# yanconglin/ICP-Flow

Measured on AMD Instinct MI355X. Metric: cluster-pair ICP registrations/sec, higher is better.
Workload: dtype f32

## Files before the change

icp_flow_amd/csrc/api.hip:

```cpp
#include <stdarg.h>
#include <stdio.h>
#include <stdlib.h>
#include <string.h>

#include "kernels.hpp"
#include "posefuse.hpp"
#include "kabsch.hpp"
#include "host.hpp"

using namespace icpflow;

namespace {

thread_local char g_err[512] = "";

}

namespace icpflow {
int report_error(int code, const char *message)
{
    snprintf(g_err, sizeof(g_err), "%s", message);
    return code;
}

// ... 920 lines not shown
    io.estimateScale = o.estimateScale;
    io.initS = o.initS;
    if ((o.allowReflection || o.estimateScale) && o.arith != ICPFLOW_ARITH_FP64)
        return report_errorf(ICPFLOW_E_ARG, "icpflow_icp: allow_reflection / estimate_scale are not built for ICPFLOW_ARITH_FP32_REFERENCE");
    if (o.history != nullptr &&
        !(stop_mode == ICPFLOW_STOP_REFERENCE && max_iterations > 1 && max_iterations <= kHistIters &&
          o.arith == ICPFLOW_ARITH_FP64 && io.speculative))
        return report_errorf(ICPFLOW_E_ARG, "icpflow_icp: options.d_icp_history needs the single-launch reference stop mode "
                                            "(2 <= max_iterations <= %d, fp64 arithmetic)", kHistIters);
    if (o.initR != nullptr && o.arith != ICPFLOW_ARITH_FP64)
        return report_errorf(ICPFLOW_E_ARG, "icpflow_icp: an initial transform is not built for ICPFLOW_ARITH_FP32_REFERENCE");
    Opts os = o;
    if ((o.estimateScale || o.initS != nullptr) && o.search == 0 && N < 64) os.search = 3;
    const GridScratch *search = search_scratch(w, N, os);
    if ((o.estimateScale || o.initS != nullptr) && (search == nullptr || search->mode != 3))
        return report_errorf(ICPFLOW_E_ARG, "icpflow_icp: estimate_scale / an initial transform with a scale need the sorted-sweep "
                                            "search (the default up to N = %d)", kMaxSortN);
    launch_count_pair(d_X, d_Y, B, N, w.lenA, w.lenC, nullptr, s, w.ctrl, icp_ctrl_bytes(B));
    ICPFLOW_TRY(launch_icp(d_X, d_Y, w.lenA, w.lenC, nullptr, d_pre_pose, B, N, thres, max_iterations,
                           relative_rmse_thr, stop_mode, w.state, w.ctrl, search, w.history, &w.team,
                           io, s));
    if (o.history != nullptr)
        ICPFLOW_TRY(hipMemcpyAsync(o.history, w.history, (size_t)max_iterations * B * kHistStride * sizeof(float),
                                   hipMemcpyDeviceToDevice, s));
    ICPFLOW_TRY(launch_icp_export(w.state, w.ctrl, B, stop_mode, d_R, d_T, d_rmse, d_iters, d_converged, s, o.scaleOut));
    return 0;
}

int icpflow_apply_icp(const float *d_src, const float *d_dst, const float *d_init, int B, int N,
                      double thres_dist, int max_iterations, double relative_rmse_thr, int stop_mode,
                      float *d_T_out, int32_t *d_iters, void *d_ws, size_t ws_bytes,
                      icpflow_stream_t stream, const icpflow_options_t *opt)
{
    Opts o;
    if (int r = parse_options("icpflow_apply_icp", opt, o)) return r;
    if (int r = check_arith("icpflow_apply_icp", o, max_iterations, stop_mode)) return r;
    if (int r = check_pair_active("icpflow_apply_icp", o, false, max_iterations, stop_mode)) return r;
    if (!d_src || !d_dst || !d_init || !d_T_out) return report_errorf(ICPFLOW_E_ARG, "icpflow_apply_icp: null pointer");
    if (int r = check_batch("icpflow_apply_icp", B, N)) return r;
    if (max_iterations <= 0 || max_iterations > kMaxIterCap)
        return report_errorf(ICPFLOW_E_ARG, "icpflow_apply_icp: max_iterations must be in 1..%d", kMaxIterCap);
    if (stop_mode != ICPFLOW_STOP_REFERENCE && stop_mode != ICPFLOW_STOP_PER_PAIR)
        return report_errorf(ICPFLOW_E_ARG, "icpflow_apply_icp: unknown stop_mode %d", stop_mode);
    Workspace w(d_ws, B, N, 0);
    if (int r = check_ws(d_ws, ws_bytes, w.bytes)) return r;
    hipStream_t s = (hipStream_t)stream;
    launch_count_pair(d_src, d_dst, B, N, w.lenA, w.lenC, nullptr, s, w.ctrl, icp_ctrl_bytes(B));
    ICPFLOW_TRY(hipMemcpyAsync(w.Tinit, d_init, (size_t)B * 16 * sizeof(float), hipMemcpyDeviceToDevice, s));
    return run_icp_and_select(d_src, d_dst, w, nullptr, w.Tinit, B, N, thres_dist, max_iterations,
                              relative_rmse_thr, stop_mode, 0, d_T_out, d_iters, o, s);
}

static int hist_icp_core(const float *d_src, const float *d_dst, int B, int N, const float *d_edges_x, int len_x,
                         const float *d_edges_y, int len_y, const float *d_edges_z, int len_z, float decode_shift,
                         double thres_dist, int max_iterations, double relative_rmse_thr, int stop_mode,
                         float *d_T_out, int32_t *d_iters, Workspace &w, const Opts &o, hipStream_t s,
                         int phase = 0, int32_t *carry = nullptr)
{
    if (phase == 2) {
        w.grid.presorted = carry[0];
        w.grid.shareCountClean = 1;
        int32_t pending = carry[2];
        return run_icp_and_select(d_src, d_dst, w, w.swap, w.Tinit, B, N, thres_dist, max_iterations,
                                  relative_rmse_thr, stop_mode, 1, d_T_out, d_iters, o, s, carry[1] != 0, 2, &pending, carry[3] != 0);
    }
    const bool countInSort = N <= kMaxSortN && N <= kChunkSortMinN && o.on(ICPFLOW_OPT_NO_SORTED_VOTE);
    if (!countInSort) {
        launch_count_pair(d_src, d_dst, B, N, w.lenA, w.lenC, w.swap, s, w.ctrl, icp_ctrl_bytes(B), w.scoreAccum,
                          w.accumBytes, w.pairBox);
        w.grid.pairBox = w.pairBox;
    }
    hipEvent_t join = nullptr;
    bool teamPlanned = false;
    JoinGuard guard;
    const GridScratch *search = search_scratch(w, N, o);
    SideStream *side = nullptr;
    if (search != nullptr && search->mode == 3 && N >= 64 && o.on(ICPFLOW_OPT_NO_SIDE_STREAM)) {
        side = &side_stream(s);
        if (!side->ok) side = nullptr;
    }
    if (side != nullptr) {
        ICPFLOW_TRY(hipEventRecord(side->fork, s));
        ICPFLOW_TRY(hipStreamWaitEvent(side->stream, side->fork, 0));
        hipError_t se = launch_sort_clouds_soa(d_src, d_dst, w.lenA, w.lenC, w.swap, B, N, &w.grid, side->stream,
                                               countInSort ? 2 : 0);
        if (se == hipSuccess && score_by_sweep(N, true, o) && o.on(ICPFLOW_OPT_NO_SCORE_PRUNE) && o.on(ICPFLOW_OPT_NO_SCORE_PREBOUND)) {
            se = launch_occupancy(&w.grid, B, N, side->stream);
            if (se == hipSuccess) w.grid.occReady = 1;
        }
        if (se == hipSuccess && !countInSort && phase != 1 &&
            icp_teams_wanted(&w.team, o.icp(w.grid.sortX), search, B, N, max_iterations, stop_mode, w.history)) {
            launch_icp_team_plan(&w.team, w.lenA, w.lenC, w.swap, B, N, o.icp(w.grid.sortX), side->stream);
            teamPlanned = true;
        }
        const hipError_t je = hipEventRecord(side->join, side->stream);
        if (je == hipSuccess) { guard.s = s; guard.join = side->join; }
        ICPFLOW_TRY(se);
        ICPFLOW_TRY(je);
        w.grid.presorted = 1;
        join = side->join;
    }
    PairCountFuse fuse{};
    if (countInSort) {
        fuse.swapOut = w.swap;
        fuse.zero0 = w.ctrl; fuse.bytes0 = icp_ctrl_bytes(B);
        fuse.zero1 = w.scoreAccum; fuse.bytes1 = w.accumBytes;
    }
    w.grid.shareCountClean = 1;
    w.grid.sweepTicket = w.ticketScratch;
    const bool sweepScore = score_by_sweep(N, join != nullptr, o);
    if (int r = run_init_pose(d_src, d_dst, w, w.swap, B, N, d_edges_x, len_x, d_edges_y, len_y, d_edges_z,
                              len_z, decode_shift, w.Tinit, o, s, sweepScore ? join : nullptr,
                              countInSort ? &fuse : nullptr, join != nullptr))
        return r;
    if (join != nullptr && !sweepScore) ICPFLOW_TRY(hipStreamWaitEvent(s, join, 0));
    guard.joined();
    if (phase == 1) {
        carry[0] = w.grid.presorted;
        carry[1] = teamPlanned ? 1 : 0;
        carry[3] = w.initSumValid ? 1 : 0;
        return run_icp_and_select(d_src, d_dst, w, w.swap, w.Tinit, B, N, thres_dist, max_iterations, relative_rmse_thr,
                                  stop_mode, 1, d_T_out, d_iters, o, s, teamPlanned, 1, &carry[2]);
    }
    return run_icp_and_select(d_src, d_dst, w, w.swap, w.Tinit, B, N, thres_dist, max_iterations,
                              relative_rmse_thr, stop_mode, 1, d_T_out, d_iters, o, s, teamPlanned, 0, nullptr, w.initSumValid);
}

int icpflow_hist_icp(const float *d_src, const float *d_dst, int B, int N, const float *d_edges_x,
                     int len_x, const float *d_edges_y, int len_y, const float *d_edges_z, int len_z,
                     float decode_shift, double thres_dist, int max_iterations, double relative_rmse_thr,
                     int stop_mode, float *d_T_out, int32_t *d_iters, void *d_ws, size_t ws_bytes,
                     icpflow_stream_t stream, const icpflow_options_t *opt)
{
    Opts o;
    if (int r = parse_options("icpflow_hist_icp", opt, o)) return r;
    if (int r = check_arith("icpflow_hist_icp", o, max_iterations, stop_mode)) return r;
    if (int r = check_pair_active("icpflow_hist_icp", o, true, max_iterations, stop_mode)) return r;
    if (!d_src || !d_dst || !d_edges_x || !d_edges_y || !d_edges_z || !d_T_out)
        return report_errorf(ICPFLOW_E_ARG, "icpflow_hist_icp: null pointer");
    if (int r = check_batch("icpflow_hist_icp", B, N)) return r;
    if (int r = check_hist_dims("icpflow_hist_icp", len_x, len_y, len_z)) return r;
    if (max_iterations <= 0 || max_iterations > kMaxIterCap)
        return report_errorf(ICPFLOW_E_ARG, "icpflow_hist_icp: max_iterations must be in 1..%d", kMaxIterCap);
    if (stop_mode != ICPFLOW_STOP_REFERENCE && stop_mode != ICPFLOW_STOP_PER_PAIR)
        return report_errorf(ICPFLOW_E_ARG, "icpflow_hist_icp: unknown stop_mode %d", stop_mode);
    const size_t L = (size_t)len_x * len_y * len_z;
    if (L < (size_t)kTopK) return report_errorf(ICPFLOW_E_ARG, "icpflow_hist_icp: fewer than 5 bins");
    Workspace w(d_ws, B, N, L);
    if (int r = check_ws(d_ws, ws_bytes, w.bytes)) return r;
    return hist_icp_core(d_src, d_dst, B, N, d_edges_x, len_x, d_edges_y, len_y, d_edges_z, len_z, decode_shift,
                         thres_dist, max_iterations, relative_rmse_thr, stop_mode, d_T_out, d_iters, w, o,
                         (hipStream_t)stream);
}

int icpflow_hist_icp_many(int K, const float *const *d_src, const float *const *d_dst, const int *B, int N,
                          const float *d_edges_x, int len_x, const float *d_edges_y, int len_y,
                          const float *d_edges_z, int len_z, float decode_shift, double thres_dist,
                          int max_iterations, double relative_rmse_thr, int stop_mode, float *const *d_T_out,
                          int32_t *const *d_iters, void *const *d_ws, const size_t *ws_bytes,
                          icpflow_stream_t stream, const icpflow_options_t *opt)
{
    if (K <= 0 || K > 64) return report_errorf(ICPFLOW_E_ARG, "icpflow_hist_icp_many: K must be in 1..64 (got %d)", K);
    if (!d_src || !d_dst || !B || !d_T_out || !d_iters || !d_ws || !ws_bytes)
        return report_errorf(ICPFLOW_E_ARG, "icpflow_hist_icp_many: null pointer");
    for (int k = 0; k < K; ++k)
        for (int j = 0; j < k; ++j)
            if (d_ws[k] == d_ws[j]) return report_errorf(ICPFLOW_E_WORKSPACE, "icpflow_hist_icp_many: batches %d and %d share a workspace", j, k);
    hipStream_t s = (hipStream_t)stream;
    constexpr int kWorkers = 4;
// ... 160 lines not shown
```

icp_flow_amd/csrc/hist.hip:

```cpp
#include "common.hpp"
#include "kernels.hpp"
#include "votekey.hpp"

namespace icpflow {

__global__ __launch_bounds__(256) void count_valid_kernel(const float4 *__restrict__ pts, int N,
                                                          int32_t *__restrict__ len)
{
    __shared__ int scratch[4];
    const int b = blockIdx.x;
    const float4 *p = pts + (size_t)b * N;
    int c[1] = {0};
    for (int i = threadIdx.x; i < N; i += blockDim.x) c[0] += (p[i].w > 0.0f) ? 1 : 0;
    block_sum<1, int>(c, scratch);
    if (threadIdx.x == 0) len[b] = c[0];
}

__global__ __launch_bounds__(1024) void count_pair_kernel(const float4 *__restrict__ A, const float4 *__restrict__ C,
                                                         int N, int32_t *__restrict__ lenA,
                                                         int32_t *__restrict__ lenC, uint8_t *__restrict__ swap,
                                                         uint32_t *__restrict__ zero0, unsigned words0,
                                                         uint32_t *__restrict__ zero1, unsigned words1,
                                                         float *__restrict__ boxes)
{
// ... 595 lines not shown
    if (useLds && N > kVoteWideN && B <= kVoteWideB * cus) {
        dim3 grid(((N + 127) / 128) * tsplit, B);
        const int lspan = (work != nullptr && N >= ICPFLOW_VOTE_LIST_MIN_N) ? min(span, kVoteListSpan) : span;
        const int ltsplit = (N + lspan - 1) / lspan;
        const size_t U = (size_t)((N + 127) / 128) * ltsplit * B;
        const bool listed = work != nullptr && U <= workCap && B <= 1024 && (N + 127) / 128 <= 256 && ltsplit <= 128 &&
                            N >= ICPFLOW_VOTE_LIST_MIN_N;
        if (listed) {
            hipLaunchKernelGGL(vote_plan_kernel, dim3((unsigned)((U + 1023) / 1024)), dim3(1024), 0, s, nX, nY, swap, B, 128, lspan,
                               (int)U, work, orderOut);
            if (planned != nullptr) *planned = orderOut != nullptr;
            grid = dim3((unsigned)U, 1);
        }
        hipLaunchKernelGGL((hist_vote_sorted_kernel<512, 4>), grid, dim3(512), lds_hist, s,
                           (const float4 *)sortX, (const float4 *)sortY, nX, nY, N, lens[0], lens[1], lens[2], ex, ey,
                           ez, swap, useLds, bins_u32, keyRec, listed ? lspan : span, listed ? work : (const int32_t *)nullptr, B);
        return hipGetLastError();
    }
    if (block == 1024) {
        dim3 grid(((N + 1023) / 1024) * tsplit, B);
        hipLaunchKernelGGL(hist_vote_sorted_kernel<1024>, grid, dim3(1024), useLds ? lds_hist : tile_bytes, s,
                           (const float4 *)sortX, (const float4 *)sortY, nX, nY, N, lens[0], lens[1], lens[2], ex, ey,
                           ez, swap, useLds, bins_u32, keyRec, span, (const int32_t *)nullptr, B);
    } else if (block == 512 && !split) {
        dim3 grid(((N + 511) / 512) * tsplit, B);
        hipLaunchKernelGGL(hist_vote_sorted_kernel<512>, grid, dim3(512), useLds ? lds_hist : tile_bytes, s,
                           (const float4 *)sortX, (const float4 *)sortY, nX, nY, N, lens[0], lens[1], lens[2], ex, ey,
                           ez, swap, useLds, bins_u32, keyRec, span, (const int32_t *)nullptr, B);
    } else if (split) {
        dim3 grid(((N + kVoteBlock - 1) / kVoteBlock) * tsplit, B);
        hipLaunchKernelGGL((hist_vote_sorted_kernel<2 * kVoteBlock, 2>), grid, dim3(2 * kVoteBlock), lds_hist, s,
                           (const float4 *)sortX, (const float4 *)sortY, nX, nY, N, lens[0], lens[1], lens[2], ex, ey,
                           ez, swap, useLds, bins_u32, keyRec, span, (const int32_t *)nullptr, B);
    } else {
        dim3 grid(((N + kVoteBlock - 1) / kVoteBlock) * tsplit, B);
        hipLaunchKernelGGL(hist_vote_sorted_kernel<kVoteBlock>, grid, dim3(kVoteBlock), useLds ? lds_hist : tile_bytes, s,
                           (const float4 *)sortX, (const float4 *)sortY, nX, nY, N, lens[0], lens[1], lens[2], ex, ey,
                           ez, swap, useLds, bins_u32, keyRec, span, (const int32_t *)nullptr, B);
    }
    return hipGetLastError();
}

__global__ void u32_to_f32_kernel(const uint32_t *__restrict__ in, float *__restrict__ out, size_t n)
{
    const size_t i = (size_t)blockIdx.x * blockDim.x + threadIdx.x;
    if (i < n) out[i] = (float)in[i];
}

hipError_t launch_hist_vote(const float *X, const float *Y, int B, int NX, int NY,
                            const float mins[3], const float maxs[3], const int lens[3],
                            const float *ex, const float *ey, const float *ez,
                            const uint8_t *swap, uint32_t *bins_u32, hipStream_t s)
{
    VoteBox box{mins ? mins[0] : 0.f, mins ? mins[1] : 0.f, mins ? mins[2] : 0.f,
                maxs ? maxs[0] : 0.f, maxs ? maxs[1] : 0.f, maxs ? maxs[2] : 0.f,
                lens[0], lens[1], lens[2]};
    const size_t L = (size_t)lens[0] * lens[1] * lens[2];
    hipError_t e = hipMemsetAsync(bins_u32, 0, sizeof(uint32_t) * L * (size_t)B, s);
    if (e != hipSuccess) return e;
    const int rows = swap ? (NX > NY ? NX : NY) : NX;
    dim3 grid((rows + kVoteBlock - 1) / kVoteBlock, B);
    const size_t tile_bytes = sizeof(float4) * kVoteTile;
    const size_t lds_hist = tile_bytes + sizeof(uint32_t) * (L + (size_t)vote_overflow_bins(lens[1], lens[2]));
    if (lds_hist <= 64 * 1024) {
        hipLaunchKernelGGL(hist_vote_kernel<true>, grid, dim3(kVoteBlock), lds_hist, s,
                           (const float4 *)X, (const float4 *)Y, NX, NY, box, ex, ey, ez, swap,
                           bins_u32);
    } else {
        hipLaunchKernelGGL(hist_vote_kernel<false>, grid, dim3(kVoteBlock), tile_bytes, s,
                           (const float4 *)X, (const float4 *)Y, NX, NY, box, ex, ey, ez, swap,
                           bins_u32);
    }
    return hipGetLastError();
}

hipError_t launch_u32_to_f32(const uint32_t *in, float *out, size_t n, hipStream_t s)
{
    hipLaunchKernelGGL(u32_to_f32_kernel, dim3((unsigned)((n + 255) / 256)), dim3(256), 0, s, in, out, n);
    return hipGetLastError();
}

constexpr int kPeakBlock = 1024;
constexpr int kPeakMaxK = 8;

template <int R>
__device__ __forceinline__ uint32_t peak_window_max(const uint32_t *__restrict__ V, int f, int c, int n, int stride)
{
    uint32_t v[2 * R + 1];
#pragma unroll
    for (int dq = -R; dq <= R; ++dq) v[dq + R] = V[f + (min(max(c + dq, 0), n - 1) - c) * stride];
    uint32_t m = v[0];
#pragma unroll
    for (int u = 1; u < 2 * R + 1; ++u) m = max(m, v[u]);
    return m;
}

#ifdef ICPFLOW_PEAK_CLOCK
__device__ unsigned long long g_peakClock[1024][8];
#define PEAK_STAMP(k) do { if (threadIdx.x == 0 && blockIdx.x < 1024) g_peakClock[blockIdx.x][k] = wall_clock64(); } while (0)
#else
#define PEAK_STAMP(k) do { } while (0)
#endif
template <typename BinT, int MEM>
__global__ __launch_bounds__(kPeakBlock) void hist_peaks_kernel(
    const BinT *__restrict__ bins, int Lx, int Ly, int Lz, int k, int radius,
    uint32_t *__restrict__ wsA, uint32_t *__restrict__ wsB, float *__restrict__ votes,
    int64_t *__restrict__ idx_out, PeakDecode dec)
{
    extern __shared__ __attribute__((aligned(16))) unsigned char smem[];
    __shared__ unsigned long long red[(kPeakBlock / kWave) * kPeakMaxK];
    __shared__ unsigned long long chosen[kPeakMaxK];
    const int b = blockIdx.x;
    const int L = Lx * Ly * Lz;
    const BinT *h = bins + (size_t)b * L;
    uint32_t *H0 = reinterpret_cast<uint32_t *>(smem);
    uint32_t *A = MEM ? H0 + L : wsA + (size_t)b * L;
    uint32_t *Bv = MEM ? H0 + 2 * (size_t)L : wsB + (size_t)b * L;
    const int tid = threadIdx.x;
    PEAK_STAMP(0);
    if (MEM) {
        for (int f = tid; f < L; f += kPeakBlock) H0[f] = (uint32_t)h[f];
        __syncthreads();
    }
    PEAK_STAMP(1);
    const int LyLz = Ly * Lz;
    const int stepX = kPeakBlock / LyLz, stepY = (kPeakBlock % LyLz) / Lz, stepZ = kPeakBlock % Lz;
    const int x0 = tid / LyLz, y0 = (tid % LyLz) / Lz, z0 = tid % Lz;
#define ICPFLOW_PEAK_ADVANCE()                                   \
    do {                                                         \
        z += stepZ; y += stepY; x += stepX;                      \
        if (z >= Lz) { z -= Lz; ++y; }                           \
        if (y >= Ly) { y -= Ly; ++x; }                           \
    } while (0)
    {
        int x = x0, y = y0, z = z0;
        for (int f = tid; f < L; f += kPeakBlock) {
            (void)x;
            uint32_t m = 0;
            if (MEM && radius >= 2 && Lz == 3) m = max(max(H0[f - z], H0[f - z + 1]), H0[f - z + 2]);
            else {
                const int lo = max(0, z - radius), hi = min(Lz - 1, z + radius);
                for (int q = lo; q <= hi; ++q) m = max(m, MEM ? H0[f + (q - z)] : (uint32_t)h[f + (q - z)]);
            }
            A[f] = m;
            ICPFLOW_PEAK_ADVANCE();
        }
    }
    __syncthreads();
    PEAK_STAMP(2);
    {
        int x = x0, y = y0, z = z0;
        for (int f = tid; f < L; f += kPeakBlock) {
            (void)x;
            uint32_t m = 0;
            if (radius == 5) m = peak_window_max<5>(A, f, y, Ly, Lz);
            else {
                const int lo = max(0, y - radius), hi = min(Ly - 1, y + radius);
                for (int q = lo; q <= hi; ++q) m = max(m, A[f + (q - y) * Lz]);
            }
            Bv[f] = m;
            ICPFLOW_PEAK_ADVANCE();
        }
    }
    __syncthreads();
    PEAK_STAMP(3);
    {
        int x = x0, y = y0, z = z0;
        for (int f = tid; f < L; f += kPeakBlock) {
            uint32_t m = 0;
            if (radius == 5) m = peak_window_max<5>(Bv, f, x, Lx, LyLz);
            else {
                const int lo = max(0, x - radius), hi = min(Lx - 1, x + radius);
                for (int q = lo; q <= hi; ++q) m = max(m, Bv[f + (q - x) * LyLz]);
            }
            A[f] = m;
            ICPFLOW_PEAK_ADVANCE();
        }
    }
#undef ICPFLOW_PEAK_ADVANCE
    __syncthreads();
    PEAK_STAMP(4);
    const int lane = tid & (kWave - 1), wave = tid >> 6;
    unsigned long long *wtop = reinterpret_cast<unsigned long long *>(red);
    {
        unsigned long long below = ~0ull, best = 0ull;
        bool stale = true;
        for (int r = 0; r < k; ++r) {
            if (stale) {
                best = 0ull;
                for (int f = tid; f < L; f += kPeakBlock) {
                    const uint32_t v = MEM ? H0[f] : (uint32_t)h[f];
                    const uint32_t sv = (v == A[f]) ? v : 0u;
                    const unsigned long long key =
                        ((unsigned long long)sv << 32) | (unsigned long long)(0xFFFFFFFFu - (uint32_t)f);
                    if (key < below && key > best) best = key;
                }
                stale = false;
            }
            const unsigned long long w = wave_max_u64_dpp(best);
            if (lane == 0) wtop[wave * kPeakMaxK + r] = w;
            if (w == best && w != 0ull) { below = best; stale = true; }
        }
    }
    __syncthreads();
    PEAK_STAMP(5);
    if (wave == 0) {
        constexpr int kWaves = kPeakBlock / kWave;
        unsigned long long c0 = 0ull, c1 = 0ull;
        {
            const int n = kWaves * k;
            if (lane < n) c0 = wtop[(lane / k) * kPeakMaxK + lane % k];
            if (lane + kWave < n) c1 = wtop[((lane + kWave) / k) * kPeakMaxK + (lane + kWave) % k];
        }
        for (int r = 0; r < k; ++r) {
            const unsigned long long m = wave_max_u64_dpp(c0 > c1 ? c0 : c1);
            if (lane == 0) chosen[r] = m;
            if (c0 == m) c0 = 0ull;
            if (c1 == m) c1 = 0ull;
        }
    }
    __syncthreads();
    PEAK_STAMP(6);
    if (tid < k) {
        const int r = tid;
        const unsigned long long m = chosen[r];
        votes[(size_t)b * k + r] = (float)(uint32_t)(m >> 32);
        const uint32_t f = 0xFFFFFFFFu - (uint32_t)(m & 0xFFFFFFFFull);
        idx_out[(size_t)b * k + r] = (int64_t)f;
        if (dec.cand != nullptr) {
            float *o = dec.cand + ((size_t)b * (k + 1) + r) * 3;
            const int ix = (int)(f / Lz / Ly % Lx), iy = (int)(f / Lz % Ly), iz = (int)(f % Lz);
            o[0] = dec.ex[ix] + dec.shift; o[1] = dec.ey[iy] + dec.shift; o[2] = dec.ez[iz] + dec.shift;
            if (r == k - 1) { o[3] = 0.f; o[4] = 0.f; o[5] = 0.f; }
        }
    }
}

template <typename BinT>
static hipError_t launch_peaks_t(const BinT *bins, int B, int Lx, int Ly, int Lz, int k,
                                 int kernel_size, uint32_t *wsA, uint32_t *wsB, float *votes,
                                 int64_t *idx, PeakDecode dec, hipStream_t s)
{
    const size_t lds = 3 * sizeof(uint32_t) * (size_t)Lx * Ly * Lz;
    if (lds <= 150 * 1024) {
        static std::atomic<unsigned long long> attr{0ull};
        ensure_dynamic_lds(reinterpret_cast<const void *>(&hist_peaks_kernel<BinT, 1>), 150 * 1024, &attr);
        hipLaunchKernelGGL((hist_peaks_kernel<BinT, 1>), dim3(B), dim3(kPeakBlock), lds, s, bins, Lx, Ly, Lz, k,
                           (kernel_size - 1) / 2, wsA, wsB, votes, idx, dec);
    } else {
        hipLaunchKernelGGL((hist_peaks_kernel<BinT, 0>), dim3(B), dim3(kPeakBlock), 0, s, bins, Lx, Ly, Lz, k,
                           (kernel_size - 1) / 2, wsA, wsB, votes, idx, dec);
    }
    return hipGetLastError();
}

hipError_t launch_hist_peaks_f32(const float *bins, int B, int Lx, int Ly, int Lz, int k,
                                 int kernel_size, uint32_t *wsA, uint32_t *wsB, float *votes,
                                 int64_t *idx, hipStream_t s)
{
    return launch_peaks_t<float>(bins, B, Lx, Ly, Lz, k, kernel_size, wsA, wsB, votes, idx, PeakDecode{}, s);
}

hipError_t launch_hist_peaks_u32(const uint32_t *bins, int B, int Lx, int Ly, int Lz, int k,
                                 int kernel_size, uint32_t *wsA, uint32_t *wsB, float *votes,
                                 int64_t *idx, hipStream_t s, PeakDecode dec)
{
    return launch_peaks_t<uint32_t>(bins, B, Lx, Ly, Lz, k, kernel_size, wsA, wsB, votes, idx, dec, s);
}

}

#ifdef ICPFLOW_PEAK_CLOCK
extern "C" int icpflow_debug_peak_clock(unsigned long long *out)
{
    (void)hipDeviceSynchronize();
    return (int)hipMemcpyFromSymbol(out, HIP_SYMBOL(icpflow::g_peakClock), sizeof(icpflow::g_peakClock));
}
#endif
```

icp_flow_amd/csrc/kernels.hpp:

```cpp
#pragma once
#include <hip/hip_runtime.h>
#include <atomic>
#include <stddef.h>
#include <stdint.h>

#include "../../include/icpflow_hip.h"

namespace icpflow {

constexpr int ICPFLOW_STOP_REFERENCE_ = ICPFLOW_STOP_REFERENCE;
constexpr int ICPFLOW_STOP_PER_PAIR_ = ICPFLOW_STOP_PER_PAIR;

constexpr int kPartial = 8;
constexpr int kMaxIterCap = 1024;
constexpr int kCand = 6;
constexpr int kTopK = 5;
constexpr int kNmsKernel = 11;

struct IcpState {
    float R[9];
    float T[3];
    float rmse;
    int active;
    int iters;
// ... 43 lines not shown
    int32_t *wgRank;
    int32_t *teamSize;
    int32_t *next;
    unsigned int *arrived;
    double *mom;
    int maxWG;
};

inline size_t icp_ctrl_bytes(int B)
{
    return sizeof(IcpCtrl) + (size_t)B * sizeof(HelpPair) + 2 * (size_t)kHelpMaxWG * sizeof(int);
}
inline IcpHelp icp_help_carve(IcpCtrl *ctrl, int B, float *state, double *out)
{
    IcpHelp h;
    h.pair = reinterpret_cast<HelpPair *>(ctrl + 1);
    h.tag = reinterpret_cast<int *>(h.pair + B);
    h.owner = h.tag + kHelpMaxWG;
    h.state = state;
    h.out = out;
    return h;
}

constexpr int kHistIters = 128;
constexpr int kHistStride = 16;

void launch_count_valid(const float *pts, int B, int N, int32_t *len, hipStream_t s);
void launch_count_pair(const float *A, const float *C, int B, int N, int32_t *lenA, int32_t *lenC, uint8_t *swap,
                       hipStream_t s, void *zero0 = nullptr, size_t bytes0 = 0, void *zero1 = nullptr, size_t bytes1 = 0,
                       float *boxes = nullptr);
hipError_t launch_hist_vote(const float *X, const float *Y, int B, int NX, int NY,
                            const float mins[3], const float maxs[3], const int lens[3],
                            const float *ex, const float *ey, const float *ez,
                            const uint8_t *swap, uint32_t *bins_u32, hipStream_t s);
struct PairCountFuse {
    uint8_t *swapOut;
    void *zero0; size_t bytes0;
    void *zero1; size_t bytes1;
};
hipError_t launch_hist_vote_sorted(const float *X, const float *Y, int32_t *nX, int32_t *nY,
                                   int B, int N, const int lens[3], const float *ex, const float *ey,
                                   const float *ez, const uint8_t *swap, float *sortX, float *sortY,
                                   uint32_t *bins_u32, float *ckey, int *cidx, float *keyRec, hipStream_t s,
                                   const PairCountFuse *fuse = nullptr, bool sideBusy = false, const float *boxes = nullptr,
                                   int32_t *work = nullptr, size_t workCap = 0, int32_t *orderOut = nullptr, bool *planned = nullptr);
size_t vote_work_capacity(int B, int N);
constexpr int kChunkSortMinN = 4096;
constexpr int kPairBoxStride = 24;
int chunk_sort_length(int N);
hipError_t launch_zsort_chunked(const float *P, const float *Q, const int32_t *nP, const int32_t *nQ, int B, int N,
                                float *outP, float *outQ, uint32_t *bins, int L, float *ckey, int *cidx,
                                const float *ez, int len_z, float *keyRec, hipStream_t s, const float *boxes = nullptr);
hipError_t launch_sort_clouds_chunked(const float *X, const float *Y, const int32_t *lenX, const int32_t *lenY,
                                      const uint8_t *swap, const float *prePose, int B, int N, int32_t *axisOut,
                                      float *Xs, float *Ys, float *Ysoa, float *Xsoa, float *ckey, int *cidx,
                                      hipStream_t s, const float *boxes = nullptr, int dirKeys = 0);
hipError_t launch_u32_to_f32(const uint32_t *in, float *out, size_t n, hipStream_t s);
hipError_t launch_hist_peaks_f32(const float *bins, int B, int Lx, int Ly, int Lz, int k,
                                 int kernel_size, uint32_t *wsA, uint32_t *wsB, float *votes,
                                 int64_t *idx, hipStream_t s);
struct PeakDecode {
    const float *ex = nullptr, *ey = nullptr, *ez = nullptr;
    float shift = 0.f;
    float *cand = nullptr;
};
hipError_t launch_hist_peaks_u32(const uint32_t *bins, int B, int Lx, int Ly, int Lz, int k,
                                 int kernel_size, uint32_t *wsA, uint32_t *wsB, float *votes,
                                 int64_t *idx, hipStream_t s, PeakDecode dec = PeakDecode{});

struct GridScratch;
hipError_t launch_sweep_pair_table(const int32_t *lenA, const int32_t *lenC, const uint8_t *swap, const int32_t *pairOrder,
                                   int B, int N, int32_t *tab, hipStream_t s);
int scan_qblocks(int maxRows, int batch);
int sweep_qblocks(int maxRows);
hipError_t launch_sweep_eval(const GridScratch *grid, const int32_t *len1, const int32_t *len2, int B, int N,
                             const float *pose, float thres, float *srcT, double *partial, hipStream_t s, const uint8_t *swap = nullptr,
                             const uint8_t *active = nullptr);
struct PoseSource;
hipError_t launch_sweep_check(const GridScratch *grid, const float *X, const float *Y, const int32_t *lenA,
                              const int32_t *lenC, const uint8_t *swap, int B, int N, const float *poseInit,
                              const float *poseFinal, double *partial, hipStream_t s, const PoseSource *fused = nullptr,
                              const uint8_t *active = nullptr, const double *initSum = nullptr);
hipError_t launch_occupancy(const GridScratch *grid, int B, int N, hipStream_t s);
hipError_t launch_sweep_score(const GridScratch *grid, const int32_t *lenA, const int32_t *lenC, const uint8_t *swap,
                              int B, int N, const float *cand, double *partial, hipStream_t s);
hipError_t launch_sweep_score_pruned(const GridScratch *grid, const int32_t *lenA, const int32_t *lenC,
                                     const uint8_t *swap, int B, int N, const float *cand, double *partial,
                                     double *accum, hipStream_t s);
hipError_t launch_scan_score(const float *A, const float *C, const int32_t *lenA, const int32_t *lenC,
                             const uint8_t *swap, int B, int N, const float *cand, double *partial,
                             hipStream_t s);
int score_qblocks(int maxRows);
hipError_t launch_scan_score_pruned(const float *A, const float *C, const int32_t *lenA, const int32_t *lenC,
                                    const uint8_t *swap, int B, int N, const float *cand, double *partial,
                                    double *accum, hipStream_t s, bool accumCleared = false);
hipError_t launch_scan_check(const float *A, const float *C, const int32_t *lenA, const int32_t *lenC,
                             const uint8_t *swap, int B, int N, const float *poseInit,
                             const float *poseFinal, double *partial, hipStream_t s);
hipError_t launch_scan_eval(const float *A, const float *C, const int32_t *lenA, const int32_t *lenC,
                            int B, int N, const float *pose, float thres, double *partial, hipStream_t s);
hipError_t launch_scan_nn(const float *Qp, const float *Tp, int B, int NQ, int NT, int strideQ,
                          int strideT, const int32_t *lenQ, const int32_t *lenT, int sqrt_dist,
                          int64_t *idx, float *dist, hipStream_t s);

constexpr int kOccWords = 1024;
#ifndef ICPFLOW_OCC_RINGS
#define ICPFLOW_OCC_RINGS 3
#endif
constexpr int kOccRings = ICPFLOW_OCC_RINGS;
constexpr int kSweepShareSlots = 16;
struct GridScratch {
    int mode;
    int H;
    float *origin;
    int32_t *start;
    int32_t *cursor;
    float *pts;
    float *sortX;
    float *sortYsoa;
    float *sortXsoa;
    int32_t *axis;
    int dirKeys;
    float *ckey;
    int *cidx;
    const float *pairBox;
    const int32_t *pairTab;
    const int32_t *pairOrder;
    float *shareBest;
    int *shareCount;
    int shareCountClean;
    float *occHdr;
    uint32_t *occBits;
    int occReady;
    int32_t *occTot;
    int *sweepTicket;
    int *scoreList;
    int presorted;
};
struct LaunchProfile;
struct IcpOpts {
    int arith = 0;
    bool teams = true;
    bool speculative = true;
    bool adaptiveWindows = true;
    bool persistent = true;
    bool helpers = true;
    IcpHelp help{};
    const float *initR = nullptr;
    const float *initT = nullptr;
    bool allowReflection = false;
    bool estimateScale = false;
    const float *initS = nullptr;
    LaunchProfile *profile = nullptr;
    bool ctrlCleared = false;
    bool *historyPending = nullptr;
    float *fp32Scratch = nullptr;
    bool teamPlanned = false;
    const uint8_t *pairActive = nullptr;
    bool teamsHalfGpu = false;
    bool sharedScans = true;
    bool twoLaunch = false;
    int32_t *splitScratch = nullptr;
};

int device_cus();
void ensure_dynamic_lds(const void *func, int bytes, std::atomic<unsigned long long> *doneMask);
// ... 104 lines not shown
```

icp_flow_amd/csrc/nn.hip:

```cpp
#include "scan.hpp"
#include "sortdir.hpp"
#include "kernels.hpp"
#include "posefuse.hpp"

namespace icpflow {

enum ScanMode : int { MODE_SCORE = 0, MODE_CHECK = 1, MODE_EVAL = 2, MODE_NN = 3 };

struct ScanParams {
    const float *A;
    const float *C;
    const int32_t *lenA;
    const int32_t *lenC;
    const uint8_t *swap;
    int N;
    int NT;
    int strideQ, strideT;
    int njobs;
    int qblocks;
    const float *cand;
    int subBegin, subCount, prune;
    double *accum;
    int split;
    const float *poseA;
// ... 957 lines not shown
        tab[k * 4 + d] = (b << 16) | (min(shares * nqb, 255) << 8) | min(nqb, 255);
    }
}

hipError_t launch_sweep_pair_table(const int32_t *lenA, const int32_t *lenC, const uint8_t *swap, const int32_t *pairOrder,
                                   int B, int N, int32_t *tab, hipStream_t s)
{
    if (B > 32767 || sweep_qblocks(N) > 255) return hipErrorInvalidValue;
    hipLaunchKernelGGL(sweep_pair_table_kernel, dim3((B + 255) / 256), dim3(256), 0, s, lenA, lenC, swap, pairOrder, B,
                       sweep_qblocks(N), tab);
    return hipGetLastError();
}

template <int MODE>
static hipError_t launch_sweep(SweepParams p, hipStream_t s)
{
    p.NP16 = (p.N + kChunk - 1) / kChunk * kChunk;
    p.qblocks = sweep_qblocks(p.N);
    p.r0 = 0.15f;
#ifndef ICPFLOW_NO_SWEEP_SHARE
    p.shareWindows = 1;
#endif
#ifdef ICPFLOW_NO_SWEEP_SHARE
    p.shareCount = nullptr;
#endif
    if (p.N < kSweepFullScanMinTargets || p.shareBest == nullptr) p.shareCount = nullptr;
    if (p.shareCount != nullptr && !p.shareClean) {
        const hipError_t me = hipMemsetAsync(p.shareCount, 0, (size_t)(MODE == SWEEP_SCORE ? (p.njobs / p.subCount) * 12 : p.njobs) * kSweepFullQb * sizeof(int), s);
        if (me != hipSuccess) return me;
    }
    const int groups = (MODE == SWEEP_CHECK && p.initSum != nullptr) ? 2 * ((p.njobs / 2 + 7) / 8) : (p.njobs + 7) / 8;
    const size_t lds = (size_t)((p.NP16 < kSweepStage ? p.NP16 : kSweepStage) * 33 / 32 + 1) * sizeof(float);
    const int total = groups * 8 * p.qblocks;
    if (MODE == SWEEP_SCORE && p.listMode == 1) {
        const int first = groups * 8;
        if (p.shareWindows != 0 && p.N >= kSweepFullScanMinTargets && p.njobs <= 12 * 700)
            hipLaunchKernelGGL((sweep_scan_kernel<MODE, true>), dim3((unsigned)first), dim3(kSweepBlock), lds, s, p);
        else
            hipLaunchKernelGGL((sweep_scan_kernel<MODE, false>), dim3((unsigned)first), dim3(kSweepBlock), lds, s, p);
        return hipGetLastError();
    }
    if (MODE == SWEEP_SCORE && p.listMode == 2) {
        const int wgs = total < 8 * 256 ? total : 8 * 256;
        if (p.shareWindows != 0 && p.N >= kSweepFullScanMinTargets && p.njobs <= 12 * 700)
            hipLaunchKernelGGL((sweep_list_kernel<MODE, true>), dim3((unsigned)wgs), dim3(kSweepBlock), lds, s, p);
        else
            hipLaunchKernelGGL((sweep_list_kernel<MODE, false>), dim3((unsigned)wgs), dim3(kSweepBlock), lds, s, p);
        return hipGetLastError();
    }
    if (MODE == SWEEP_SCORE && p.pairSlots > 0) {
        const unsigned blocks = (unsigned)((p.njobs / p.subCount) * (p.qblocks * p.pairSlots + 10 - p.pairSlots));
        if (p.shareWindows != 0 && p.N >= kSweepFullScanMinTargets && p.njobs <= 12 * 700)
            hipLaunchKernelGGL((sweep_pair_kernel<true>), dim3(blocks), dim3(kSweepBlock), lds, s, p);
        else
            hipLaunchKernelGGL((sweep_pair_kernel<false>), dim3(blocks), dim3(kSweepBlock), lds, s, p);
        return hipGetLastError();
    }
    unsigned blocks = (unsigned)total;
    if (MODE == SWEEP_SCORE && p.totBase != 0) {
        p.totBase = total;
        blocks += (unsigned)((p.njobs / p.subCount) * 10);
    }
    if (p.shareWindows != 0 && p.N >= kSweepFullScanMinTargets && p.njobs <= 12 * 700)
        hipLaunchKernelGGL((sweep_scan_kernel<MODE, true>), dim3(blocks), dim3(kSweepBlock), lds, s, p);
    else
        hipLaunchKernelGGL((sweep_scan_kernel<MODE, false>), dim3(blocks), dim3(kSweepBlock), lds, s, p);
    return hipGetLastError();
}

constexpr int kOccBlock = 256;
__device__ __forceinline__ uint32_t occ_shifted(const uint32_t *in, int w, int sh, bool up)
{
    const int q = sh >> 5, r = sh & 31;
    if (up) {
        const int a = w - q;
        const uint32_t lo = a >= 0 ? in[a] : 0u, lo1 = a - 1 >= 0 ? in[a - 1] : 0u;
        return r == 0 ? lo : ((lo << r) | (lo1 >> (32 - r)));
    }
    const int a = w + q;
    const uint32_t hi = a < kOccWords ? in[a] : 0u, hi1 = a + 1 < kOccWords ? in[a + 1] : 0u;
    return r == 0 ? hi : ((hi >> r) | (hi1 << (32 - r)));
}

__global__ __launch_bounds__(kOccBlock) void occ_build_kernel(const float *__restrict__ Xsoa, const float *__restrict__ Ysoa,
                                                            int NP16, float *__restrict__ hdrOut, uint32_t *__restrict__ bitsOut)
{
    __shared__ uint32_t bitsA[kOccWords], bitsB[kOccWords];
    __shared__ float red[6 * (kOccBlock / kWave)];
    __shared__ float hd[8];
    const int b = blockIdx.x, which = blockIdx.y, tid = threadIdx.x, lane = tid & (kWave - 1), wave = tid >> 6;
    const float *px = (which == 0 ? Xsoa : Ysoa) + (size_t)b * 3 * NP16, *py = px + NP16, *pz = py + NP16;
    for (int k = tid; k < kOccWords; k += kOccBlock) bitsA[k] = 0u;
    float mn[3] = {kInf, kInf, kInf}, mx[3] = {-kInf, -kInf, -kInf};
    for (int i = tid; i < NP16; i += kOccBlock) {
        const float x = px[i], y = py[i], z = pz[i];
        if (fabsf(x) < 1e30f && fabsf(y) < 1e30f && fabsf(z) < 1e30f) {
            mn[0] = fminf(mn[0], x); mn[1] = fminf(mn[1], y); mn[2] = fminf(mn[2], z);
            mx[0] = fmaxf(mx[0], x); mx[1] = fmaxf(mx[1], y); mx[2] = fmaxf(mx[2], z);
        }
    }
#pragma unroll
    for (int a = 0; a < 3; ++a) {
#pragma unroll
        for (int o = kWave / 2; o > 0; o >>= 1) {
            mn[a] = fminf(mn[a], __shfl_xor(mn[a], o, kWave));
            mx[a] = fmaxf(mx[a], __shfl_xor(mx[a], o, kWave));
        }
        if (lane == 0) { red[wave * 6 + a] = mn[a]; red[wave * 6 + 3 + a] = mx[a]; }
    }
    __syncthreads();
    if (tid == 0) {
        float lo[3], hi[3];
        for (int a = 0; a < 3; ++a) {
            lo[a] = kInf; hi[a] = -kInf;
            for (int w = 0; w < kOccBlock / kWave; ++w) { lo[a] = fminf(lo[a], red[w * 6 + a]); hi[a] = fmaxf(hi[a], red[w * 6 + 3 + a]); }
        }
        int n[3] = {0, 0, 0};
        float h = 0.125f;
        if (lo[0] <= hi[0]) {
            for (int grow = 0; grow < 64; ++grow) {
                bool fits = true;
                long long cells = 1;
                for (int a = 0; a < 3; ++a) {
                    const float e = (hi[a] - lo[a]) / h;
                    if (!(e < 30000.f)) { fits = false; break; }
                    n[a] = (int)e + 2 + 2 * kOccRings;
                    cells *= n[a];
                }
                if (fits && cells <= (long long)kOccWords * 32) break;
                h *= 1.25f; n[0] = 0;
            }
        }
        if (n[0] <= 0) n[0] = n[1] = n[2] = 0;
        hd[0] = lo[0] - kOccRings * h; hd[1] = lo[1] - kOccRings * h; hd[2] = lo[2] - kOccRings * h;
        float big = 0.f;
        for (int a = 0; a < 3; ++a) big = fmaxf(big, fmaxf(fabsf(lo[a]), fabsf(hi[a])));
        if (!(big * 2.4e-7f / h < 0.005f)) n[0] = n[1] = n[2] = 0;
        hd[3] = 1.0f / h; hd[4] = 0.98f * h;
        hd[5] = __int_as_float(n[0]); hd[6] = __int_as_float(n[1]); hd[7] = __int_as_float(n[2]);
    }
    __syncthreads();
    const float gox = hd[0], goy = hd[1], goz = hd[2], ginv = hd[3];
    const int gnx = __float_as_int(hd[5]), gny = __float_as_int(hd[6]), gnz = __float_as_int(hd[7]);
    if (gnx > 0) {
        for (int i = tid; i < NP16; i += kOccBlock) {
            const float x = px[i], y = py[i], z = pz[i];
            if (!(fabsf(x) < 1e30f && fabsf(y) < 1e30f && fabsf(z) < 1e30f)) continue;
            const int cx = min(max((int)floorf((x - gox) * ginv), kOccRings), gnx - 1 - kOccRings);
            const int cy = min(max((int)floorf((y - goy) * ginv), kOccRings), gny - 1 - kOccRings);
            const int cz = min(max((int)floorf((z - goz) * ginv), kOccRings), gnz - 1 - kOccRings);
            const int c = (cx * gny + cy) * gnz + cz;
            atomicOr(&bitsA[c >> 5], 1u << (c & 31));
        }
    }
    __syncthreads();
    const int strides[3] = {1, gnz, gny * gnz};
    uint32_t *in = bitsA, *outb = bitsB;
    uint32_t *bo = bitsOut + ((size_t)b * 2 + which) * kOccRings * kOccWords;
    for (int ring = 0; ring < kOccRings; ++ring) {
        for (int a = 0; a < 3; ++a) {
            if (gnx > 0)
                for (int w = tid; w < kOccWords; w += kOccBlock) outb[w] = in[w] | occ_shifted(in, w, strides[a], true) | occ_shifted(in, w, strides[a], false);
            __syncthreads();
            uint32_t *t = in; in = outb; outb = t;
        }
        for (int k = tid; k < kOccWords; k += kOccBlock) bo[ring * kOccWords + k] = gnx > 0 ? in[k] : 0u;
    }
    if (tid < 8) hdrOut[((size_t)b * 2 + which) * 8 + tid] = hd[tid];
}

hipError_t launch_occupancy(const GridScratch *grid, int B, int N, hipStream_t s)
{
    if (grid->occHdr == nullptr || grid->occBits == nullptr || grid->sortXsoa == nullptr || grid->sortYsoa == nullptr) return hipSuccess;
    const int NP16 = (N + kChunk - 1) / kChunk * kChunk;
    hipLaunchKernelGGL(occ_build_kernel, dim3(B, 2), dim3(kOccBlock), 0, s, grid->sortXsoa, grid->sortYsoa, NP16, grid->occHdr, grid->occBits);
    return hipGetLastError();
}

hipError_t launch_sweep_score(const GridScratch *grid, const int32_t *lenA, const int32_t *lenC, const uint8_t *swap,
                              int B, int N, const float *cand, double *partial, hipStream_t s)
{
    SweepParams p{};
    p.Asoa = grid->sortXsoa; p.Csoa = grid->sortYsoa; p.lenA = lenA; p.lenC = lenC; p.swap = swap;
    p.axis = grid->axis; p.cand = cand; p.N = N; p.njobs = B * 12; p.partial = partial;
    p.subBegin = 0; p.subCount = 12;
    p.shareBest = grid->shareBest; p.shareCount = grid->shareCount; p.shareClean = grid->shareCountClean; p.pairOrder = grid->pairOrder; p.pairTab = grid->pairTab;
    return launch_sweep<SWEEP_SCORE>(p, s);
}

hipError_t launch_sweep_score_pruned(const GridScratch *grid, const int32_t *lenA, const int32_t *lenC,
                                     const uint8_t *swap, int B, int N, const float *cand, double *partial,
                                     double *accum, hipStream_t s)
{
    SweepParams p{};
    p.Asoa = grid->sortXsoa; p.Csoa = grid->sortYsoa; p.lenA = lenA; p.lenC = lenC; p.swap = swap;
    p.axis = grid->axis; p.cand = cand; p.N = N; p.partial = partial; p.accum = accum;
    if (grid->occReady) { p.occHdr = grid->occHdr; p.occBits = grid->occBits; }
    p.shareBest = grid->shareBest; p.shareCount = grid->shareCount; p.shareClean = grid->shareCountClean; p.pairOrder = grid->pairOrder; p.pairTab = grid->pairTab;
    if (grid->occReady) {
#ifndef ICPFLOW_SCORE_LIST_MIN_JOBS
#define ICPFLOW_SCORE_LIST_MIN_JOBS 65536
#endif
        const bool listed = grid->sweepTicket != nullptr && grid->scoreList != nullptr &&
                            (long long)B * 10 * sweep_qblocks(N) >= ICPFLOW_SCORE_LIST_MIN_JOBS;
#ifndef ICPFLOW_SCORE_PAIR_MAX_BLOCKS
#define ICPFLOW_SCORE_PAIR_MAX_BLOCKS 1024
#endif
#ifndef ICPFLOW_SCORE_PAIR_WHOLE_MAX_QBLOCKS
#define ICPFLOW_SCORE_PAIR_WHOLE_MAX_QBLOCKS 4
#endif
        const bool byPair = kSweepPairSlots > 0 && !listed && grid->occTot != nullptr && (long long)B * sweep_qblocks(N) <= ICPFLOW_SCORE_PAIR_MAX_BLOCKS;
        p.njobs = B * 2; p.subBegin = 0; p.subCount = 2; p.prune = 0;
        if (byPair) { p.occTot = grid->occTot; p.totBase = 1; }
        hipError_t e2 = launch_sweep<SWEEP_SCORE>(p, s);
        if (e2 != hipSuccess) return e2;
        p.totBase = 0;
        p.njobs = B * 10; p.subBegin = 2; p.subCount = 10; p.prune = 1; p.boundBoth = 1;
        if (byPair) {
            p.pairSlots = sweep_qblocks(N) <= ICPFLOW_SCORE_PAIR_WHOLE_MAX_QBLOCKS ? kSweepPairSlots : 10;
            return launch_sweep<SWEEP_SCORE>(p, s);
        }
        if (listed) {
            p.list = grid->scoreList; p.listCount = grid->sweepTicket;
            p.listMode = 1;
            const hipError_t e3 = launch_sweep<SWEEP_SCORE>(p, s);
            if (e3 != hipSuccess) return e3;
            p.listMode = 2;
        }
        return launch_sweep<SWEEP_SCORE>(p, s);
    }
    p.njobs = B; p.subBegin = 0; p.subCount = 1; p.prune = 0;
    hipError_t e = launch_sweep<SWEEP_SCORE>(p, s);
    if (e != hipSuccess) return e;
    p.njobs = B * 11; p.subBegin = 1; p.subCount = 11; p.prune = 1;
    return launch_sweep<SWEEP_SCORE>(p, s);
}

hipError_t launch_sweep_eval(const GridScratch *grid, const int32_t *len1, const int32_t *len2, int B, int N,
                             const float *pose, float thres, float *srcT, double *partial, hipStream_t s,
                             const uint8_t *swap, const uint8_t *active)
{
    SweepParams p{};
    p.active = active;
    p.Asoa = grid->sortXsoa; p.Csoa = grid->sortYsoa; p.lenA = len1; p.lenC = len2; p.axis = grid->axis;
    p.swap = swap;
    p.poseA = pose; p.thres = thres; p.srcT = srcT; p.N = N; p.njobs = B * 2; p.partial = partial;
    p.shareBest = grid->shareBest; p.shareCount = grid->shareCount; p.shareClean = grid->shareCountClean; p.pairOrder = grid->pairOrder; p.pairTab = grid->pairTab;
    const int NP16 = (N + kChunk - 1) / kChunk * kChunk;
    hipLaunchKernelGGL(transform_soa_kernel, dim3((NP16 + 255) / 256, B), dim3(256), 0, s, grid->sortXsoa, len1, pose,
                       NP16, srcT, grid->sortYsoa, swap);
    return launch_sweep<SWEEP_EVAL>(p, s);
}

hipError_t launch_sweep_check(const GridScratch *grid, const float *X, const float *Y, const int32_t *lenA,
                              const int32_t *lenC, const uint8_t *swap, int B, int N, const float *poseInit,
                              const float *poseFinal, double *partial, hipStream_t s, const PoseSource *fused,
                              const uint8_t *active, const double *initSum)
{
// ... 106 lines not shown
```

Baseline: 411,000.

## Restructure peak finding with line-segment max filters and survivor list; build occupancy before sort

The histogram peak kernel now fuses the load with the z-axis max, computes the y/x window maxima with a van Herk style prefix/suffix line pass, and collects local-maximum survivors into a compact shared list so one wave selects the top-k. This is meant to cut redundant window reads and the full-grid per-wave top-k reduction. Separately, on the side stream for small N, the occupancy grid is built directly from the raw float4 clouds (optionally counting valid points itself) before the sort, rather than waiting for the sorted SoA. The list path falls back to the old reduction when there are too many survivors, and the raw occupancy path reads only the valid rows, which assumes valid points come first in each cloud.

```diff
diff --git a/icp_flow_amd/csrc/api.hip b/icp_flow_amd/csrc/api.hip
--- a/icp_flow_amd/csrc/api.hip
+++ b/icp_flow_amd/csrc/api.hip
@@ -1026,9 +1026,16 @@
     if (side != nullptr) {
         ICPFLOW_TRY(hipEventRecord(side->fork, s));
         ICPFLOW_TRY(hipStreamWaitEvent(side->stream, side->fork, 0));
-        hipError_t se = launch_sort_clouds_soa(d_src, d_dst, w.lenA, w.lenC, w.swap, B, N, &w.grid, side->stream,
-                                               countInSort ? 2 : 0);
-        if (se == hipSuccess && score_by_sweep(N, true, o) && o.on(ICPFLOW_OPT_NO_SCORE_PRUNE) && o.on(ICPFLOW_OPT_NO_SCORE_PREBOUND)) {
+        const bool wantOcc = score_by_sweep(N, true, o) && o.on(ICPFLOW_OPT_NO_SCORE_PRUNE) && o.on(ICPFLOW_OPT_NO_SCORE_PREBOUND);
+        const bool occFirst = wantOcc && N <= kChunkSortMinN;
+        hipError_t se = hipSuccess;
+        if (occFirst) {
+            se = launch_occupancy_raw(d_src, d_dst, w.lenA, w.lenC, w.swap, B, N, &w.grid, countInSort ? 2 : 0, side->stream);
+            if (se == hipSuccess) w.grid.occReady = 1;
+        }
+        if (se == hipSuccess)
+            se = launch_sort_clouds_soa(d_src, d_dst, w.lenA, w.lenC, w.swap, B, N, &w.grid, side->stream, countInSort ? 2 : 0);
+        if (se == hipSuccess && wantOcc && !occFirst) {
             se = launch_occupancy(&w.grid, B, N, side->stream);
             if (se == hipSuccess) w.grid.occReady = 1;
         }
diff --git a/icp_flow_amd/csrc/hist.hip b/icp_flow_amd/csrc/hist.hip
--- a/icp_flow_amd/csrc/hist.hip
+++ b/icp_flow_amd/csrc/hist.hip
@@ -701,6 +701,10 @@
 
 constexpr int kPeakBlock = 1024;
 constexpr int kPeakMaxK = 8;
+constexpr int kPeakList = 512;
+#ifndef ICPFLOW_PEAK_PARTS
+#define ICPFLOW_PEAK_PARTS 7
+#endif
 
 template <int R>
 __device__ __forceinline__ uint32_t peak_window_max(const uint32_t *__restrict__ V, int f, int c, int n, int stride)
@@ -712,6 +716,25 @@
 #pragma unroll
     for (int u = 1; u < 2 * R + 1; ++u) m = max(m, v[u]);
     return m;
+}
+
+template <int R>
+__device__ __forceinline__ void peak_line_max(const uint32_t *__restrict__ src, uint32_t *__restrict__ dst, int base, int stride,
+                                              int n, int s0)
+{
+    uint32_t v[4 * R + 1];
+#pragma unroll
+    for (int j = 0; j <= 4 * R; ++j) v[j] = src[base + min(max(s0 - R + j, 0), n - 1) * stride];
+    uint32_t suf[2 * R + 1], pre[2 * R + 1];
+    suf[2 * R] = v[2 * R];
+#pragma unroll
+    for (int j = 2 * R - 1; j >= 0; --j) suf[j] = max(v[j], suf[j + 1]);
+    pre[0] = v[2 * R];
+#pragma unroll
+    for (int j = 1; j <= 2 * R; ++j) pre[j] = max(pre[j - 1], v[2 * R + j]);
+#pragma unroll
+    for (int i = 0; i <= 2 * R; ++i)
+        if (s0 + i < n) dst[base + (s0 + i) * stride] = max(suf[i], pre[i]);
 }
 
 #ifdef ICPFLOW_PEAK_CLOCK
@@ -726,9 +749,13 @@
     uint32_t *__restrict__ wsA, uint32_t *__restrict__ wsB, float *__restrict__ votes,
     int64_t *__restrict__ idx_out, PeakDecode dec)
 {
+    constexpr bool kFillZ = MEM != 0 && (ICPFLOW_PEAK_PARTS & 1) != 0, kLines = MEM != 0 && (ICPFLOW_PEAK_PARTS & 2) != 0,
+                   kList = MEM != 0 && (ICPFLOW_PEAK_PARTS & 4) != 0;
     extern __shared__ __attribute__((aligned(16))) unsigned char smem[];
-    __shared__ unsigned long long red[(kPeakBlock / kWave) * kPeakMaxK];
+    __shared__ unsigned long long red[kList ? kPeakList : (kPeakBlock / kWave) * kPeakMaxK];
     __shared__ unsigned long long chosen[kPeakMaxK];
+    __shared__ unsigned int nSurvivors;
+    static_assert(kPeakList >= (kPeakBlock / kWave) * kPeakMaxK, "the waves' keys reuse the list");
     const int b = blockIdx.x;
     const int L = Lx * Ly * Lz;
     const BinT *h = bins + (size_t)b * L;
@@ -737,7 +764,31 @@
     uint32_t *Bv = MEM ? H0 + 2 * (size_t)L : wsB + (size_t)b * L;
     const int tid = threadIdx.x;
     PEAK_STAMP(0);
-    if (MEM) {
+    if (kList && tid == 0) nSurvivors = 0u;
+    if (kFillZ) {
+        const int nCol = Lx * Ly;
+        for (int c = tid; c < nCol; c += kPeakBlock) {
+            const int f0 = c * Lz;
+            if (Lz == 3 && radius >= 2) {
+                const uint32_t v0 = (uint32_t)h[f0], v1 = (uint32_t)h[f0 + 1], v2 = (uint32_t)h[f0 + 2];
+                const uint32_t m = max(max(v0, v1), v2);
+                H0[f0] = v0; H0[f0 + 1] = v1; H0[f0 + 2] = v2;
+                A[f0] = m; A[f0 + 1] = m; A[f0 + 2] = m;
+            } else if (Lz <= 2 * radius + 1) {
+                uint32_t m = 0;
+                for (int z = 0; z < Lz; ++z) { const uint32_t v = (uint32_t)h[f0 + z]; H0[f0 + z] = v; m = max(m, v); }
+                for (int z = 0; z < Lz; ++z) A[f0 + z] = m;
+            } else {
+                for (int z = 0; z < Lz; ++z) H0[f0 + z] = (uint32_t)h[f0 + z];
+                for (int z = 0; z < Lz; ++z) {
+                    const int lo = max(0, z - radius), hi = min(Lz - 1, z + radius);
+                    uint32_t m = 0;
+                    for (int q = lo; q <= hi; ++q) m = max(m, H0[f0 + q]);
+                    A[f0 + z] = m;
+                }
+            }
+        }
+    } else if (MEM) {
         for (int f = tid; f < L; f += kPeakBlock) H0[f] = (uint32_t)h[f];
         __syncthreads();
     }
@@ -751,7 +802,7 @@
         if (z >= Lz) { z -= Lz; ++y; }                           \
         if (y >= Ly) { y -= Ly; ++x; }                           \
     } while (0)
-    {
+    if (!kFillZ) {
         int x = x0, y = y0, z = z0;
         for (int f = tid; f < L; f += kPeakBlock) {
             (void)x;
@@ -767,7 +818,27 @@
     }
     __syncthreads();
     PEAK_STAMP(2);
-    {
+    const bool lines = kLines && radius == 5;
+    if (lines) {
+        constexpr int W = 2 * 5 + 1;
+        {
+            const int nLines = Lx * Lz, items = nLines * ((Ly + W - 1) / W);
+            for (int it = tid; it < items; it += kPeakBlock) {
+                const int seg = it / nLines, line = it - seg * nLines, x = line / Lz, z = line - x * Lz;
+                peak_line_max<5>(A, Bv, x * LyLz + z, Lz, Ly, seg * W);
+            }
+        }
+        __syncthreads();
+        PEAK_STAMP(3);
+        {
+            const int items = LyLz * ((Lx + W - 1) / W);
+            for (int it = tid; it < items; it += kPeakBlock) {
+                const int seg = it / LyLz, line = it - seg * LyLz;
+                peak_line_max<5>(Bv, A, line, LyLz, Lx, seg * W);
+            }
+        }
+    }
+    if (!lines) {
         int x = x0, y = y0, z = z0;
         for (int f = tid; f < L; f += kPeakBlock) {
             (void)x;
@@ -781,9 +852,11 @@
             ICPFLOW_PEAK_ADVANCE();
         }
     }
-    __syncthreads();
-    PEAK_STAMP(3);
-    {
+    if (!lines) {
+        __syncthreads();
+        PEAK_STAMP(3);
+    }
+    if (!lines) {
         int x = x0, y = y0, z = z0;
         for (int f = tid; f < L; f += kPeakBlock) {
             uint32_t m = 0;
@@ -800,8 +873,54 @@
     __syncthreads();
     PEAK_STAMP(4);
     const int lane = tid & (kWave - 1), wave = tid >> 6;
+    bool listed = false;
+    if constexpr (kList) {
+        for (int f0 = wave * kWave; f0 < L; f0 += kPeakBlock) {
+            const int f = f0 + lane;
+            uint32_t v = 0u;
+            bool surv = false;
+            if (f < L) { v = H0[f]; surv = v != 0u && v == A[f]; }
+            const unsigned long long mask = __ballot(surv);
+            if (mask != 0ull) {
+                unsigned int at = 0u;
+                if (lane == 0) at = atomicAdd(&nSurvivors, (unsigned int)__popcll(mask));
+                at = (unsigned int)__builtin_amdgcn_readfirstlane((int)at) + (unsigned int)__popcll(mask & ((1ull << lane) - 1ull));
+                if (surv && at < (unsigned int)kPeakList)
+                    red[at] = ((unsigned long long)v << 32) | (unsigned long long)(0xFFFFFFFFu - (uint32_t)f);
+            }
+        }
+        __syncthreads();
+        PEAK_STAMP(5);
+        const int n = (int)nSurvivors;
+        listed = n <= kPeakList;
+        if (listed && wave == 0) {
+            unsigned long long below = ~0ull, best = 0ull;
+            bool stale = true;
+            const int top = min(n, k);
+            for (int r = 0; r < top; ++r) {
+                if (stale) {
+                    best = 0ull;
+                    for (int j = lane; j < n; j += kWave) {
+                        const unsigned long long key = red[j];
+                        if (key < below && key > best) best = key;
+                    }
+                    stale = false;
+                }
+                const unsigned long long w = wave_max_u64_dpp(best);
+                if (lane == 0) chosen[r] = w;
+                if (w == best && w != 0ull) { below = best; stale = true; }
+            }
+            if (n < k) {
+                bool zero = false;
+                if (lane < L) { const uint32_t v = H0[lane]; zero = !(v != 0u && v == A[lane]); }
+                const unsigned long long mask = __ballot(zero);
+                const int rank = __popcll(mask & ((1ull << lane) - 1ull));
+                if (zero && rank < k - n) chosen[n + rank] = (unsigned long long)(0xFFFFFFFFu - (uint32_t)lane);
+            }
+        }
+    }
     unsigned long long *wtop = reinterpret_cast<unsigned long long *>(red);
-    {
+    if (!listed) {
         unsigned long long below = ~0ull, best = 0ull;
         bool stale = true;
         for (int r = 0; r < k; ++r) {
@@ -821,9 +940,9 @@
             if (w == best && w != 0ull) { below = best; stale = true; }
         }
     }
-    __syncthreads();
-    PEAK_STAMP(5);
-    if (wave == 0) {
+    if (!listed) __syncthreads();
+    if (!kList) PEAK_STAMP(5);
+    if (!listed && wave == 0) {
         constexpr int kWaves = kPeakBlock / kWave;
         unsigned long long c0 = 0ull, c1 = 0ull;
         {
diff --git a/icp_flow_amd/csrc/kernels.hpp b/icp_flow_amd/csrc/kernels.hpp
--- a/icp_flow_amd/csrc/kernels.hpp
+++ b/icp_flow_amd/csrc/kernels.hpp
@@ -149,6 +149,8 @@
                               const float *poseFinal, double *partial, hipStream_t s, const PoseSource *fused = nullptr,
                               const uint8_t *active = nullptr, const double *initSum = nullptr);
 hipError_t launch_occupancy(const GridScratch *grid, int B, int N, hipStream_t s);
+hipError_t launch_occupancy_raw(const float *X, const float *Y, const int32_t *lenX, const int32_t *lenY, const uint8_t *swap, int B, int N,
+                                const GridScratch *grid, int selfCount, hipStream_t s);
 hipError_t launch_sweep_score(const GridScratch *grid, const int32_t *lenA, const int32_t *lenC, const uint8_t *swap,
                               int B, int N, const float *cand, double *partial, hipStream_t s);
 hipError_t launch_sweep_score_pruned(const GridScratch *grid, const int32_t *lenA, const int32_t *lenC,
diff --git a/icp_flow_amd/csrc/nn.hip b/icp_flow_amd/csrc/nn.hip
--- a/icp_flow_amd/csrc/nn.hip
+++ b/icp_flow_amd/csrc/nn.hip
@@ -1063,18 +1063,48 @@
     return r == 0 ? hi : ((hi >> r) | (hi1 << (32 - r)));
 }
 
+template <bool RAW>
 __global__ __launch_bounds__(kOccBlock) void occ_build_kernel(const float *__restrict__ Xsoa, const float *__restrict__ Ysoa,
-                                                            int NP16, float *__restrict__ hdrOut, uint32_t *__restrict__ bitsOut)
+                                                            int NP16, float *__restrict__ hdrOut, uint32_t *__restrict__ bitsOut,
+                                                            const int32_t *__restrict__ lenX, const int32_t *__restrict__ lenY,
+                                                            const uint8_t *__restrict__ swap, int selfCount)
 {
     __shared__ uint32_t bitsA[kOccWords], bitsB[kOccWords];
     __shared__ float red[6 * (kOccBlock / kWave)];
     __shared__ float hd[8];
     const int b = blockIdx.x, which = blockIdx.y, tid = threadIdx.x, lane = tid & (kWave - 1), wave = tid >> 6;
-    const float *px = (which == 0 ? Xsoa : Ysoa) + (size_t)b * 3 * NP16, *py = px + NP16, *pz = py + NP16;
+    const float *px, *py, *pz;
+    int rows = NP16;
+    constexpr int kStep = RAW ? 4 : 1;
+    if (RAW) {
+        int cX, cY;
+        bool sw;
+        if (selfCount) {
+            __shared__ int cntScratch[2 * (kOccBlock / kWave)];
+            const float4 *qx = reinterpret_cast<const float4 *>(Xsoa) + (size_t)b * NP16;
+            const float4 *qy = reinterpret_cast<const float4 *>(Ysoa) + (size_t)b * NP16;
+            int c[2] = {0, 0};
+            for (int i = tid; i < NP16; i += kOccBlock) {
+                c[0] += (qx[i].w > 0.0f) ? 1 : 0;
+                c[1] += (qy[i].w > 0.0f) ? 1 : 0;
+            }
+            block_sum<2, int>(c, cntScratch);
+            cX = c[0]; cY = c[1];
+            sw = selfCount == 2 && cX > cY;
+        } else {
+            cX = lenX[b]; cY = lenY[b];
+            sw = swap != nullptr && swap[b] != 0;
+        }
+        const bool fromY = (which == 0) == sw;
+        px = (fromY ? Ysoa : Xsoa) + (size_t)b * NP16 * 4; py = px + 1; pz = px + 2;
+        rows = fromY ? cY : cX;
+    } else {
+        px = (which == 0 ? Xsoa : Ysoa) + (size_t)b * 3 * NP16; py = px + NP16; pz = py + NP16;
+    }
     for (int k = tid; k < kOccWords; k += kOccBlock) bitsA[k] = 0u;
     float mn[3] = {kInf, kInf, kInf}, mx[3] = {-kInf, -kInf, -kInf};
-    for (int i = tid; i < NP16; i += kOccBlock) {
-        const float x = px[i], y = py[i], z = pz[i];
+    for (int i = tid; i < rows; i += kOccBlock) {
+        const float x = px[i * kStep], y = py[i * kStep], z = pz[i * kStep];
         if (fabsf(x) < 1e30f && fabsf(y) < 1e30f && fabsf(z) < 1e30f) {
             mn[0] = fminf(mn[0], x); mn[1] = fminf(mn[1], y); mn[2] = fminf(mn[2], z);
             mx[0] = fmaxf(mx[0], x); mx[1] = fmaxf(mx[1], y); mx[2] = fmaxf(mx[2], z);
@@ -1124,8 +1154,8 @@
     const float gox = hd[0], goy = hd[1], goz = hd[2], ginv = hd[3];
     const int gnx = __float_as_int(hd[5]), gny = __float_as_int(hd[6]), gnz = __float_as_int(hd[7]);
     if (gnx > 0) {
-        for (int i = tid; i < NP16; i += kOccBlock) {
-            const float x = px[i], y = py[i], z = pz[i];
+        for (int i = tid; i < rows; i += kOccBlock) {
+            const float x = px[i * kStep], y = py[i * kStep], z = pz[i * kStep];
             if (!(fabsf(x) < 1e30f && fabsf(y) < 1e30f && fabsf(z) < 1e30f)) continue;
             const int cx = min(max((int)floorf((x - gox) * ginv), kOccRings), gnx - 1 - kOccRings);
             const int cy = min(max((int)floorf((y - goy) * ginv), kOccRings), gny - 1 - kOccRings);
@@ -1154,7 +1184,16 @@
 {
     if (grid->occHdr == nullptr || grid->occBits == nullptr || grid->sortXsoa == nullptr || grid->sortYsoa == nullptr) return hipSuccess;
     const int NP16 = (N + kChunk - 1) / kChunk * kChunk;
-    hipLaunchKernelGGL(occ_build_kernel, dim3(B, 2), dim3(kOccBlock), 0, s, grid->sortXsoa, grid->sortYsoa, NP16, grid->occHdr, grid->occBits);
+    hipLaunchKernelGGL(occ_build_kernel<false>, dim3(B, 2), dim3(kOccBlock), 0, s, grid->sortXsoa, grid->sortYsoa, NP16, grid->occHdr, grid->occBits,
+                       (const int32_t *)nullptr, (const int32_t *)nullptr, (const uint8_t *)nullptr, 0);
+    return hipGetLastError();
+}
+
+hipError_t launch_occupancy_raw(const float *X, const float *Y, const int32_t *lenX, const int32_t *lenY, const uint8_t *swap, int B, int N,
+                                const GridScratch *grid, int selfCount, hipStream_t s)
+{
+    if (grid->occHdr == nullptr || grid->occBits == nullptr || grid->sortXsoa == nullptr || grid->sortYsoa == nullptr) return hipSuccess;
+    hipLaunchKernelGGL(occ_build_kernel<true>, dim3(B, 2), dim3(kOccBlock), 0, s, X, Y, N, grid->occHdr, grid->occBits, lenX, lenY, swap, selfCount);
     return hipGetLastError();
 }
 
```

Measured after the change: 419,800 (median of 6 runs). +2.1%, better.
